# fundamentalvision/BEVFormer

Hardware: NVIDIA H100
Metric: BEV queries/sec (bevformer_base 200x200x256, 6 cams) fwd+bwd (higher is better)
Workload: dtype bf16

## Files before the change

### bevformer_b200/_lib.py

```python
from __future__ import annotations

import ctypes
import os
import threading

from . import build as _build

_lock = threading.Lock()
_lib = None

c_void_p, c_int, c_int64 = ctypes.c_void_p, ctypes.c_int, ctypes.c_int64

SIGNATURES = {
    "bevf_version": (c_int, []),
    "bevf_last_error": (ctypes.c_char_p, []),
    "bevf_launch_count": (c_int64, []),
    "bevf_msda_forward": (c_int, [c_void_p, c_int, c_void_p, c_void_p, c_void_p, c_void_p,
                                  c_void_p, c_int] + [c_int] * 7 + [c_void_p]),
    "bevf_msda_backward": (c_int, [c_void_p, c_int, c_void_p, c_void_p, c_void_p, c_void_p,
                                   c_void_p, c_int, c_void_p, c_void_p, c_void_p] + [c_int] * 7
                           + [c_void_p]),
    "bevf_msda_rows_forward": (c_int, [c_void_p, c_int, c_void_p, c_void_p, c_void_p, c_void_p,
                                       c_void_p, c_int, c_void_p] + [c_int] * 7 + [c_void_p]),
    "bevf_msda_rows_backward": (c_int, [c_void_p, c_int, c_void_p, c_void_p, c_void_p, c_void_p,
# ... 58 lines not shown
    "bevf_sca_combine_forward": (c_int, [c_void_p] * 4 + [c_int] * 6 + [c_void_p]),
    "bevf_sca_combine_backward": (c_int, [c_void_p] * 4 + [c_int] * 5 + [c_void_p]),
    "bevf_linear_forward": (c_int, [c_void_p] * 3 + [c_int] + [c_void_p] * 2
                            + [c_int, c_int64, c_int, c_int, c_int, c_void_p]),
    "bevf_flatten_feats": (c_int, [c_void_p] * 4 + [c_int] * 7 + [c_void_p]),
    "bevf_linear_dgrad": (c_int, [c_void_p] * 3 + [c_int64, c_int, c_int, c_void_p]),
    "bevf_linear_dgrad_acc": (c_int, [c_void_p] * 4 + [c_int64, c_int, c_int, c_void_p]),
    "bevf_linear_wgrad": (c_int, [c_void_p] * 4 + [c_int64, c_int, c_int, c_void_p]),
    "bevf_linear_wgrad_workspace_bytes": (c_int64, [c_int64, c_int, c_int]),
    "bevf_linear_wgrad_out": (c_int, [c_void_p] * 4 + [c_int, c_void_p, c_int64, c_int64, c_int, c_int,
                                                      c_void_p]),
    "bevf_sum_tensors": (c_int, [c_void_p, c_int, c_void_p, c_int64, c_int, c_void_p]),
    "bevf_linear_wgrad_into": (c_int, [c_void_p] * 5 + [c_int64, c_int64, c_int, c_int, c_void_p]),
    "bevf_linear_forward_dt": (c_int, [c_void_p] * 3 + [c_int] + [c_void_p] * 2
                               + [c_int, c_int64, c_int, c_int, c_int, c_int, c_void_p]),
    "bevf_linear_dgrad_dt": (c_int, [c_void_p] * 3 + [c_int64, c_int, c_int, c_int, c_void_p]),
    "bevf_linear_dgrad_acc_dt": (c_int, [c_void_p] * 4 + [c_int64, c_int, c_int, c_int, c_void_p]),
    "bevf_linear_wgrad_dt": (c_int, [c_void_p] * 4 + [c_int64, c_int, c_int, c_int, c_void_p]),
    "bevf_linear_wgrad_out_dt": (c_int, [c_void_p] * 4 + [c_int, c_void_p, c_int64, c_int64, c_int, c_int, c_int,
                                                         c_void_p]),
    "bevf_linear_wgrad_into_dt": (c_int, [c_void_p] * 5 + [c_int64, c_int64, c_int, c_int, c_int, c_void_p]),
    "bevf_colsum": (c_int, [c_void_p, c_void_p, c_int64, c_int, c_int, c_void_p]),
    "bevf_colsum_workspace_bytes": (c_int64, [c_int64, c_int]),
    "bevf_colsum_det": (c_int, [c_void_p, c_void_p, c_void_p, c_int64, c_int64, c_int, c_int, c_void_p]),
    "bevf_dropout_inplace": (c_int, [c_void_p, c_int64, ctypes.c_float, ctypes.c_uint64, c_void_p, c_int,
                                     c_void_p]),
    "bevf_relu_dropout_backward": (c_int, [c_void_p, c_void_p, c_void_p, c_int64, ctypes.c_float, c_int,
                                           c_void_p]),
    "bevf_point_sampling": (c_int, [c_void_p, c_void_p, c_void_p, ctypes.c_float, ctypes.c_float,
                                    c_void_p, c_void_p] + [c_int] * 5 + [c_void_p]),
# ... 64 lines not shown
```

### bevformer_b200/csrc/gemm.cu

```cuda
#include <cuda.h>

#include <cstdlib>
#include <cstring>
#include <type_traits>

#include "common.cuh"
#include "wgmma.cuh"

namespace bevf {

constexpr int kBM = 128;
constexpr int kBK = 64;
constexpr int kGemmThreads = 384;
constexpr int kChunk = 64 * 128;
constexpr int kMaxStages = 6;

__device__ __forceinline__ float load_bias(const void *bias, int dt, int col) {
    if (dt == BEVF_DTYPE_BF16) return __bfloat162float(reinterpret_cast<const bf16 *>(bias)[col]);
    if (dt == BEVF_DTYPE_F16) return __half2float(reinterpret_cast<const __half *>(bias)[col]);
    return reinterpret_cast<const float *>(bias)[col];
}

struct GemmParams {
    int M, N;
// ... 185 lines not shown
                if (p.red) {
                    float *dst = reinterpret_cast<float *>(p.y) + off;
                    asm volatile("red.global.add.v2.f32 [%0], {%1, %2};" ::"l"(dst), "f"(v0), "f"(v1) : "memory");
                } else if (p.out_f32) {
                    *reinterpret_cast<float2 *>(reinterpret_cast<float *>(p.y) + off) = make_float2(v0, v1);
                } else {
                    *reinterpret_cast<uint32_t *>(reinterpret_cast<TE *>(p.y) + off) = St16<TE>::pack(v0, v1);
                }
            }
        }
    }
}

constexpr int kWsRows = 64;
constexpr int kWsBoxBytes = 64 * 128;
constexpr int kWsStageMax = 4 * kWsBoxBytes;
constexpr int kWsWeightMax = 128 * 1024;

struct WsParams {
    int M, N, R;
    int tiles_m, tiles_n, groups;
    int stages;
    int stg_bytes;
    int relu;
    const void *bias;
    int bias_dt;
    int addend;
    int out_f32;
};

__device__ __forceinline__ void tma_store_2d(const CUtensorMap *map, const void *src, int c0, int c1) {
    asm volatile("cp.async.bulk.tensor.2d.global.shared::cta.bulk_group [%0, {%2, %3}], [%1];"
                 ::"l"(map), "r"(smem_u32(src)), "r"(c0), "r"(c1) : "memory");
}

template <int BN, bool kBmn, typename TE>
__global__ void __launch_bounds__(kGemmThreads, 1)
gemm_ws_wgmma(const __grid_constant__ CUtensorMap map_a, const __grid_constant__ CUtensorMap map_w,
              const __grid_constant__ CUtensorMap map_y, const __grid_constant__ CUtensorMap map_add,
              const WsParams p) {
    static_assert(BN == 64 || BN == 128 || BN == 256, "tile width");
    extern __shared__ __align__(1024) uint8_t smem_raw[];
    uint8_t *smem = reinterpret_cast<uint8_t *>((reinterpret_cast<uintptr_t>(smem_raw) + 1023) & ~uintptr_t(1023));
    const int kblocks = p.R / kBK;
    const int w_bytes = kblocks * BN * 128;
    uint8_t *sw = smem;
    uint8_t *stg0 = sw + w_bytes;
    uint8_t *ring0 = stg0 + 2 * p.stg_bytes;
    uint64_t *bars = reinterpret_cast<uint64_t *>(ring0 + 2 * p.stages * kWsBoxBytes);
    uint64_t *w_full = bars;
    uint64_t *full = bars + 1, *empty = full + 2 * kMaxStages;
    uint64_t *add_full = empty + 2 * kMaxStages, *stg_empty = add_full + 2;
    float *sbias = reinterpret_cast<float *>(stg_empty + 2);

    const int wg = threadIdx.x >> 7, warp = threadIdx.x >> 5, lane = threadIdx.x & 31;
    const int tn = blockIdx.x % p.tiles_n, g = blockIdx.x / p.tiles_n;
    const int t_begin = (int)((int64_t)g * p.tiles_m / p.groups);
    const int t_end = (int)((int64_t)(g + 1) * p.tiles_m / p.groups);
    const int col0 = tn * BN;

    if (threadIdx.x == 0) {
        asm volatile("prefetch.tensormap [%0];" ::"l"(&map_a) : "memory");
        asm volatile("prefetch.tensormap [%0];" ::"l"(&map_w) : "memory");
        asm volatile("prefetch.tensormap [%0];" ::"l"(&map_y) : "memory");
        mbar_init(w_full, 1);
        for (int i = 0; i < 2 * kMaxStages; ++i) { mbar_init(&full[i], 1); mbar_init(&empty[i], 4); }
        for (int i = 0; i < 2; ++i) { mbar_init(&add_full[i], 1); mbar_init(&stg_empty[i], 1); }
        asm volatile("fence.mbarrier_init.release.cluster;" ::: "memory");
    }
    __syncthreads();

    if (wg == 0) {
        asm volatile("setmaxnreg.dec.sync.aligned.u32 40;\n" ::: "memory");
        if (warp < 2 && lane == 0) {
            const int c = warp;
            if (c == 0) {
                const int chunks = kBmn ? min(BN / 64, (p.N - col0 + 63) / 64) : 1;
                mbar_expect_tx(w_full, (uint32_t)(kblocks * (kBmn ? chunks * kChunk : BN * 128)));
                for (int kb = 0; kb < kblocks; ++kb) {
                    uint8_t *dst = sw + (size_t)kb * BN * 128;
                    if (!kBmn) {
                        tma_load_2d(dst, &map_w, w_full, kb * kBK, col0);
                    } else {
                        for (int ch = 0; ch < chunks; ++ch)
                            tma_load_2d(dst + ch * kChunk, &map_w, w_full, col0 + ch * 64, kb * kBK);
                    }
                }
            }
            uint8_t *ring = ring0 + (size_t)c * p.stages * kWsBoxBytes, *stg = stg0 + (size_t)c * p.stg_bytes;
            uint64_t *f = full + c * kMaxStages, *e = empty + c * kMaxStages;
            const int add_boxes = min(BN / 64, (p.N - col0 + 63) / 64);
            int s = 0; uint32_t ph = 0, t = 0;
            for (int tm = t_begin + c; tm < t_end; tm += 2, ++t) {
                for (int kb = 0; kb < kblocks; ++kb) {
                    mbar_wait(&e[s], ph ^ 1);
                    mbar_expect_tx(&f[s], (uint32_t)kWsBoxBytes);
                    tma_load_2d(ring + (size_t)s * kWsBoxBytes, &map_a, &f[s], kb * kBK, tm * kWsRows);
                    if (++s == p.stages) { s = 0; ph ^= 1; }
                }
                if (p.addend) {
                    if (t > 0) mbar_wait(&stg_empty[c], (t - 1) & 1);
                    mbar_expect_tx(&add_full[c], (uint32_t)(add_boxes * kWsBoxBytes));
                    for (int b = 0; b < add_boxes; ++b)
                        tma_load_2d(stg + b * kWsBoxBytes, &map_add, &add_full[c], col0 + b * 64, tm * kWsRows);
                }
            }
        }
        return;
    }
    asm volatile("setmaxnreg.inc.sync.aligned.u32 232;\n" ::: "memory");

    const int cw = wg - 1, w4 = warp & 3;
    const bool leader = (threadIdx.x & 127) == 0;
    uint8_t *ring = ring0 + (size_t)cw * p.stages * kWsBoxBytes, *stg = stg0 + (size_t)cw * p.stg_bytes;
    uint64_t *f = full + cw * kMaxStages, *e = empty + cw * kMaxStages;
    constexpr int kF32PassCols = BN > 128 ? 128 : BN;
    const int passes = p.out_f32 ? BN / kF32PassCols : 1;
    const uint32_t sw_base = smem_u32(sw);
    constexpr uint64_t db_step = kBmn ? 128 : 2;
    float acc[BN / 2];
    for (int i = threadIdx.x - 128; i < BN; i += 256) {
        const int col = col0 + i;
        float b = 0.f;
        if (p.bias && col < p.N) b = load_bias(p.bias, p.bias_dt, col);
        sbias[i] = b;
    }
    asm volatile("bar.sync 3, 256;" ::: "memory");
    mbar_wait(w_full, 0);
    int s = 0; uint32_t ph = 0, t = 0;
    for (int tm = t_begin + cw; tm < t_end; tm += 2, ++t) {
        int prev = -1;
        for (int kb = 0; kb < kblocks; ++kb) {
            mbar_wait(&f[s], ph);
            const uint64_t da = smem_desc_sw128(smem_u32(ring + (size_t)s * kWsBoxBytes), 0);
            const uint64_t db = smem_desc_sw128(sw_base + (uint32_t)(kb * BN * 128), kChunk);
            wgmma_fence();
#pragma unroll
            for (int k = 0; k < kBK / 16; ++k)
                Wgmma<BN, 0, kBmn, TE>::run(acc, da + 2 * k, db + db_step * k, (kb | k) != 0);
            wgmma_commit();
            if (prev >= 0) {
                asm volatile("wgmma.wait_group.sync.aligned 1;" ::: "memory");
                __syncwarp();
                if (lane == 0) mbar_arrive(&e[prev]);
            }
            prev = s;
            if (++s == p.stages) { s = 0; ph ^= 1; }
// ... 10 lines not shown
            const float2 bv = *reinterpret_cast<const float2 *>(sbias + 8 * j + cq);
            const float b0 = bv.x, b1 = bv.y;
#pragma unroll
            for (int h = 0; h < 2; ++h) {
                float v0 = acc[4 * j + 2 * h] + b0, v1 = acc[4 * j + 2 * h + 1] + b1;
                if (p.relu) { v0 = fmaxf(v0, 0.f); v1 = fmaxf(v1, 0.f); }
                if (p.addend) {
                    const int r = r0 + 8 * h;
                    const uint32_t a2 = *reinterpret_cast<const uint32_t *>(
                        stg + (j >> 3) * kWsBoxBytes + r * 128 + (((j & 7) ^ (r & 7)) << 4) + 2 * cq);
                    v0 += St16<TE>::lo(a2); v1 += St16<TE>::hi(a2);
                }
                acc[4 * j + 2 * h] = v0; acc[4 * j + 2 * h + 1] = v1;
            }
        }
#pragma unroll
        for (int pass = 0; pass < 2; ++pass) {
            if (pass == passes) break;
            asm volatile("bar.sync %0, 128;" ::"r"(1 + cw) : "memory");
#pragma unroll
            for (int j = 0; j < BN / 8; ++j) {
#pragma unroll
                for (int h = 0; h < 2; ++h) {
                    const int r = r0 + 8 * h;
                    const float v0 = acc[4 * j + 2 * h], v1 = acc[4 * j + 2 * h + 1];
                    if (p.out_f32) {
                        if (j * 8 / kF32PassCols != pass) continue;
                        const int jj = j - pass * (kF32PassCols / 8);
                        const int unit = 2 * (jj & 3) + (cq >> 2);
                        *reinterpret_cast<float2 *>(stg + (jj >> 2) * kWsBoxBytes + r * 128 + ((unit ^ (r & 7)) << 4) +
                                                    4 * (cq & 3)) = make_float2(v0, v1);
                    } else {
                        *reinterpret_cast<uint32_t *>(stg + (j >> 3) * kWsBoxBytes + r * 128 +
                                                      (((j & 7) ^ (r & 7)) << 4) + 2 * cq) = St16<TE>::pack(v0, v1);
                    }
                }
            }
            asm volatile("fence.proxy.async.shared::cta;" ::: "memory");
            asm volatile("bar.sync %0, 128;" ::"r"(1 + cw) : "memory");
            if (leader) {
                const int cols_per_box = p.out_f32 ? 32 : 64, pc0 = col0 + pass * (BN / passes);
                for (int b = 0; b < BN / passes / cols_per_box && pc0 + b * cols_per_box < p.N; ++b)
                    tma_store_2d(&map_y, stg + b * kWsBoxBytes, pc0 + b * cols_per_box, tm * kWsRows);
                asm volatile("cp.async.bulk.commit_group;" ::: "memory");
                asm volatile("cp.async.bulk.wait_group.read 0;" ::: "memory");
            }
        }
        if (leader && p.addend) mbar_arrive(&stg_empty[cw]);
    }
    if (leader) asm volatile("cp.async.bulk.wait_group 0;" ::: "memory");
}

template <typename TO, bool kAcc = false>
__global__ void __launch_bounds__(256)
wgrad_reduce_kernel(const float *__restrict__ ws, const float *__restrict__ ws_b, TO *__restrict__ dw,
                    TO *__restrict__ db, int N, int K, int n_pad, int splits) {
    static_assert(!kAcc || sizeof(TO) == 4, "accumulation into fp32 only");
    const int kv = K / 4;
    const long long t = (long long)blockIdx.x * blockDim.x + threadIdx.x;
    const long long total = (long long)N * kv;
    if (t < total) {
        const int n = (int)(t / kv), c = (int)(t % kv) * 4;
        float4 a = make_float4(0.f, 0.f, 0.f, 0.f);
// ... 46 lines not shown
    const uint32_t esz = f32 ? 4 : 2;
    cuuint64_t dims[2] = {cols, rows};
    cuuint64_t strides[1] = {cols * esz};
    cuuint32_t box[2] = {128 / esz, box_rows};
    cuuint32_t estr[2] = {1, 1};
    const CUtensorMapDataType ty = f32 ? CU_TENSOR_MAP_DATA_TYPE_FLOAT32
                                 : dt == BEVF_DTYPE_F16 ? CU_TENSOR_MAP_DATA_TYPE_FLOAT16 : CU_TENSOR_MAP_DATA_TYPE_BFLOAT16;
    CUresult r = encode(map, ty, 2,
                        const_cast<void *>(ptr), dims,
                        strides, box, estr, CU_TENSOR_MAP_INTERLEAVE_NONE,
                        CU_TENSOR_MAP_SWIZZLE_128B, CU_TENSOR_MAP_L2_PROMOTION_L2_256B,
                        CU_TENSOR_MAP_FLOAT_OOB_FILL_NONE);
    return r == CUDA_SUCCESS ? 0 : (int)r;
}

template <int BN, bool kAmn, bool kBmn, typename TE>
static int launch_gemm(const char *who, const CUtensorMap &map_a, const CUtensorMap &map_b, GemmParams p,
                       cudaStream_t st) {
    constexpr int kStageBytes = kBM * 128 + BN * 128;
    int stages = (227 * 1024 - 1024 - 256) / kStageBytes;
    if (stages > kMaxStages) stages = kMaxStages;
    p.stages = stages;
    const size_t smem = 1024 + (size_t)stages * kStageBytes + 2 * kMaxStages * 8;
    static bool configured = false;
    if (!configured) {
        if (cudaFuncSetAttribute(gemm_bf16_wgmma<BN, kAmn, kBmn, TE>, cudaFuncAttributeMaxDynamicSharedMemorySize,
                                 (int)smem) != cudaSuccess) {
            cudaGetLastError();
            return fail("%s: cannot reserve shared memory for the GEMM", who);
        }
        configured = true;
    }
    const int units = ((p.M + kBM - 1) / kBM) * ((p.N + BN - 1) / BN) * p.splits;
    const int grid = units < device_sms() ? units : device_sms();
    gemm_bf16_wgmma<BN, kAmn, kBmn, TE><<<grid, kGemmThreads, smem, st>>>(map_a, map_b, p);
    return check_launch(who);
}

static int ws_block(int N, int R) {
    int bn = 256;
    while (bn > 64 && (bn * R * 2 > kWsWeightMax || bn / 2 >= N)) bn /= 2;
    return bn * R * 2 <= kWsWeightMax ? bn : 0;
}

template <int BN, bool kBmn, typename TE>
static int launch_ws(const char *who, const CUtensorMap &map_a, const CUtensorMap &map_w, const CUtensorMap &map_y,
                     const CUtensorMap &map_add, WsParams p, cudaStream_t st) {
    constexpr int kSmemMax = 227 * 1024;
    constexpr int kBarBytes = (1 + 4 * kMaxStages + 4) * 8 + BN * 4;
    p.stg_bytes = kWsRows * BN * (p.out_f32 ? 4 : 2);
    if (p.stg_bytes > kWsStageMax) p.stg_bytes = kWsStageMax;
    const int w_bytes = p.R * BN * 2;
    int stages = (kSmemMax - 1024 - kBarBytes - w_bytes - 2 * p.stg_bytes) / (2 * kWsBoxBytes);
    if (stages > kMaxStages) stages = kMaxStages;
    if (stages < 2) return fail("%s: no room for a two-stage A ring next to the weight tile", who);
    p.stages = stages;
    const size_t smem = 1024 + (size_t)w_bytes + 2 * p.stg_bytes + 2 * (size_t)stages * kWsBoxBytes + kBarBytes;
    static bool configured = false;
    if (!configured) {
        if (cudaFuncSetAttribute(gemm_ws_wgmma<BN, kBmn, TE>, cudaFuncAttributeMaxDynamicSharedMemorySize, kSmemMax) !=
            cudaSuccess) {
            cudaGetLastError();
            return fail("%s: cannot reserve shared memory for the GEMM", who);
        }
        configured = true;
    }
    p.tiles_m = (p.M + kWsRows - 1) / kWsRows;
    p.tiles_n = (p.N + BN - 1) / BN;
    p.groups = device_sms() / p.tiles_n;
    if (p.groups > p.tiles_m) p.groups = p.tiles_m;
    if (p.groups < 1) p.groups = 1;
    gemm_ws_wgmma<BN, kBmn, TE><<<p.groups * p.tiles_n, kGemmThreads, smem, st>>>(map_a, map_w, map_y, map_add, p);
    return check_launch(who);
}

template <typename TE> constexpr int dtype_of() { return std::is_same<TE, __half>::value ? BEVF_DTYPE_F16 : BEVF_DTYPE_BF16; }

template <typename TE>
static int linear_ws(const char *who, int bn, bool b_mn, const void *a, const void *w, const void *bias, int bias_dt,
                     const void *addend, void *y, bool out_f32, int M, int N, int R, int relu, cudaStream_t st) {
    constexpr int dt = dtype_of<TE>();
    CUtensorMap map_a, map_w, map_y, map_add;
    if (int e = make_map_2d(&map_a, a, (uint64_t)M, (uint64_t)R, kWsRows, dt))
        return fail("%s: cuTensorMapEncodeTiled(A) failed (%lld)", who, e);
    if (int e = b_mn ? make_map_2d(&map_w, w, (uint64_t)R, (uint64_t)N, 64, dt)
                     : make_map_2d(&map_w, w, (uint64_t)N, (uint64_t)R, (uint32_t)bn, dt))
        return fail("%s: cuTensorMapEncodeTiled(B) failed (%lld)", who, e);
    if (int e = make_map_2d(&map_y, y, (uint64_t)M, (uint64_t)N, kWsRows, out_f32 ? BEVF_DTYPE_F32 : dt))
        return fail("%s: cuTensorMapEncodeTiled(Y) failed (%lld)", who, e);
    map_add = map_y;
    if (addend)
        if (int e = make_map_2d(&map_add, addend, (uint64_t)M, (uint64_t)N, kWsRows, dt))
            return fail("%s: cuTensorMapEncodeTiled(addend) failed (%lld)", who, e);
    WsParams p;
    memset(&p, 0, sizeof(p));
    p.M = M; p.N = N; p.R = R;
    p.relu = relu; p.bias = bias; p.bias_dt = bias_dt;
    p.addend = addend != nullptr; p.out_f32 = out_f32;
    switch (bn * 2 + (int)b_mn) {
        case 512: return launch_ws<256, false, TE>(who, map_a, map_w, map_y, map_add, p, st);
        case 513: return launch_ws<256, true, TE>(who, map_a, map_w, map_y, map_add, p, st);
        case 256: return launch_ws<128, false, TE>(who, map_a, map_w, map_y, map_add, p, st);
        case 257: return launch_ws<128, true, TE>(who, map_a, map_w, map_y, map_add, p, st);
        case 128: return launch_ws<64, false, TE>(who, map_a, map_w, map_y, map_add, p, st);
        case 129: return launch_ws<64, true, TE>(who, map_a, map_w, map_y, map_add, p, st);
    }
    return fail("%s: no weight-stationary tile for this shape", who);
}

static GemmParams base_params(int M, int N, int R) {
    GemmParams p;
    memset(&p, 0, sizeof(p));
    p.M = M; p.N = N; p.R = R; p.rows_per_split = ((R + kBK - 1) / kBK) * kBK; p.splits = 1;
    p.ldy = N;
    return p;
}
// ... 3 lines not shown
using namespace bevf;

static bool operand_dtype_ok(int dtype) { return dtype == BEVF_DTYPE_BF16 || dtype == BEVF_DTYPE_F16; }

template <typename TE>
static int linear_dgrad_impl(const char *who, const void *dy, const void *w, const void *addend, void *dx, int64_t M,
                             int N, int K, void *stream) {
    constexpr int dt = dtype_of<TE>();
    if (M < 0 || N <= 0 || K <= 0) return fail("%s: bad dimension", who);
    if (M == 0) return 0;
    if (!dy || !w || !dx) return fail("%s: null pointer argument", who);
    if (N % kBK != 0 || K % 64 != 0) return fail("%s: N and K must be multiples of 64 (got %lld, %lld)", who, N, K);
    if (M >= (1ll << 31)) return fail("%s: M too large", who);
    if (!aligned16(dy) || !aligned16(w) || !aligned16(dx)) return fail("%s: pointers must be 16-byte aligned", who);
    cudaStream_t st = (cudaStream_t)stream;
    if (int bn = ws_block(K, N))
        return linear_ws<TE>(who, bn, true, dy, w, nullptr, BEVF_DTYPE_F32, addend, dx, false, (int)M, K, N, 0, st);
    CUtensorMap map_a, map_b;
    if (int e = make_map_2d(&map_a, dy, (uint64_t)M, (uint64_t)N, kBM, dt))
        return fail("%s: cuTensorMapEncodeTiled(A) failed (%lld)", who, e);
    if (int e = make_map_2d(&map_b, w, (uint64_t)N, (uint64_t)K, 64, dt))
        return fail("%s: cuTensorMapEncodeTiled(B) failed (%lld)", who, e);
    GemmParams p = base_params((int)M, K, N);
    p.addend = addend;
    p.y = dx;
    return K % 128 == 0 ? launch_gemm<128, false, true, TE>(who, map_a, map_b, p, st)
                        : launch_gemm<64, false, true, TE>(who, map_a, map_b, p, st);
}

static int linear_dgrad_dispatch(const char *who, const void *dy, const void *w, const void *addend, void *dx,
                                 int64_t M, int N, int K, int dtype, void *stream) {
// ... 28 lines not shown
                               void *stream) {
    constexpr int dt = dtype_of<TE>();
    if (M < 0 || N <= 0 || K <= 0) return fail("%s: bad dimension", who);
    if (M == 0) return 0;
    if (!x || !w || !y) return fail("%s: null pointer argument", who);
    if (K % kBK != 0) return fail("%s: K must be a multiple of 64 (got %lld)", who, K);
    if (N % 16 != 0) return fail("%s: N must be a multiple of 16 (got %lld)", who, N);
    if (M >= (1ll << 31)) return fail("%s: M too large", who);
    if (!aligned16(x) || !aligned16(w) || !aligned16(y) || (bias && !aligned16(bias)) ||
        (residual && !aligned16(residual)))
        return fail("%s: pointers must be 16-byte aligned", who);
    if (y_dtype != dt && y_dtype != BEVF_DTYPE_F32) return fail("%s: unsupported dtype code", who);
    if (bias && bias_dtype != dt && bias_dtype != BEVF_DTYPE_F32)
        return fail("%s: unsupported bias dtype code", who);
    cudaStream_t st = (cudaStream_t)stream;
    if (int bn = ws_block(N, K))
        return linear_ws<TE>(who, bn, false, x, w, bias, bias_dtype, residual, y, y_dtype == BEVF_DTYPE_F32, (int)M, N,
                             K, relu, st);
    const bool wide = N > 64;
    CUtensorMap map_a, map_b;
    if (int e = make_map_2d(&map_a, x, (uint64_t)M, (uint64_t)K, kBM, dt))
        return fail("%s: cuTensorMapEncodeTiled(A) failed (%lld)", who, e);
    if (int e = make_map_2d(&map_b, w, (uint64_t)N, (uint64_t)K, wide ? 128 : 64, dt))
        return fail("%s: cuTensorMapEncodeTiled(B) failed (%lld)", who, e);
    GemmParams p = base_params((int)M, N, K);
    p.relu = relu; p.bias = bias; p.bias_dt = bias_dtype;
    p.addend = residual;
    p.y = y; p.out_f32 = y_dtype == BEVF_DTYPE_F32;
    return wide ? launch_gemm<128, false, false, TE>(who, map_a, map_b, p, st)
                : launch_gemm<64, false, false, TE>(who, map_a, map_b, p, st);
}
// ... 2 lines not shown
                                      const void *residual, void *y, int y_dtype, int64_t M, int N, int K, int relu,
                                      int dtype, void *stream) {
    const char *who = "bevf_linear_forward_dt";
    if (dtype == BEVF_DTYPE_F16)
        return linear_forward_impl<__half>(who, x, w, bias, bias_dtype, residual, y, y_dtype, M, N, K, relu, stream);
    if (dtype == BEVF_DTYPE_BF16)
        return linear_forward_impl<bf16>(who, x, w, bias, bias_dtype, residual, y, y_dtype, M, N, K, relu, stream);
    return fail("%s: unsupported operand dtype code (bf16 or fp16)", who);
}

extern "C" int bevf_linear_forward(const void *x, const void *w, const void *bias, int bias_dtype,
                                   const void *residual, void *y, int y_dtype, int64_t M, int N, int K,
                                   int relu, void *stream) {
    return linear_forward_impl<bf16>("bevf_linear_forward", x, w, bias, bias_dtype, residual, y, y_dtype, M, N, K,
                                     relu, stream);
}

static void wgrad_plan(int64_t M, int N, int K, int &bn, int &splits, int &rows, int &n_pad) {
    bn = K % 128 == 0 ? 128 : 64;
    const int tiles_m = (N + kBM - 1) / kBM;
    const int tiles = tiles_m * (K / bn);
    splits = (device_sms() + tiles - 1) / tiles;
    rows = (int)((M + splits - 1) / splits);
    rows = ((rows + 63) / 64) * 64;
    splits = (int)((M + rows - 1) / rows);
    n_pad = tiles_m * kBM;
}

template <typename TE>
static int launch_wgrad(const char *who, const void *dy, const void *x, GemmParams p, int bn, cudaStream_t st) {
// ... 113 lines not shown
```

### bevformer_b200/ops.py

```python
from __future__ import annotations

import os
import warnings

import torch
from torch.autograd.function import Function, once_differentiable

from . import _lib

F32, BF16, F16 = 0, 1, 2
_DT = {torch.float32: F32, torch.bfloat16: BF16, torch.float16: F16}
TC_DTYPES = (torch.bfloat16, torch.float16)


def deterministic() -> bool:
    return torch.are_deterministic_algorithms_enabled()


def alert_not_deterministic(name: str) -> None:
    if not torch.are_deterministic_algorithms_enabled():
        return
    msg = (f"{name} does not have a deterministic implementation, but you set "
           "'torch.use_deterministic_algorithms(True)'.")
    if torch.is_deterministic_algorithms_warn_only_enabled():
# ... 942 lines not shown
    _need_cuda(x, "x")
    if x.dtype not in TC_DTYPES or weight.dtype != x.dtype:
        raise RuntimeError("linear_tc: x and weight must be both bfloat16 or both float16")
    K = x.shape[-1]
    N = weight.shape[0]
    M = x.numel() // K
    w = weight.contiguous()
    bq, bdt = (None, F32) if bias is None else _param_ptr(bias, x.dtype)
    res = None if residual is None else residual.contiguous()
    out_dtype = out_dtype or x.dtype
    y = torch.empty(x.shape[:-1] + (N,), device=x.device, dtype=out_dtype)
    lib = _lib.load()
    with torch.cuda.device(x.device):
        st = lib.bevf_linear_forward_dt(x.data_ptr(), w.data_ptr(), _ptr(bq), bdt, _ptr(res), y.data_ptr(),
                                        _DT[out_dtype], M, N, K, int(bool(relu)), _DT[x.dtype], _stream_ptr(x))
    _lib.check(st, lib)
    return y


def linear_dgrad_tc(dy, weight, addend=None):
    _need_cuda(dy, "dy")
    if dy.dtype not in TC_DTYPES or weight.dtype != dy.dtype or dy.shape[-1] != weight.shape[0]:
        raise RuntimeError("linear_dgrad_tc: dy (M,N) and weight (N,K) must be both bfloat16 or both float16")
    N, K = weight.shape
    if N % 64 or K % 64 or os.environ.get("BEVF_DGRAD", "mn") == "copy":
        dx = linear_tc(dy, weight.t().contiguous())
        return dx if addend is None else dx + addend.view(dx.shape)
    dy = dy.contiguous()
    w = weight.contiguous()
    M = dy.numel() // N
# ... 465 lines not shown
```

### bevformer_b200/plugin/linear.py

```python
from __future__ import annotations

import os

import torch
import torch.nn.functional as F
from torch.autograd.function import Function, once_differentiable

from .. import ops
from ..arena import arena_of


def _use_tc(x: torch.Tensor, weight: torch.Tensor) -> bool:
    return (x.is_cuda and x.dtype in ops.TC_DTYPES and weight.shape[1] % 64 == 0
            and weight.shape[0] % 16 == 0 and os.environ.get("BEVF_GEMM", "tc") != "cublas")


def stacked_head(weights, biases, x):
    from ..arena import stacked
    n, k = sum(w.shape[0] for w in weights), weights[0].shape[1]
    direct = (x.is_cuda and x.dtype in ops.TC_DTYPES and k % 64 == 0 and n % 16 == 0
              and os.environ.get("BEVF_GEMM", "tc") != "cublas")
    return stacked(weights, direct), stacked(biases, direct)


# ... 86 lines not shown


class _SharedInputProjections(Function):

    @staticmethod
    def forward(ctx, state, x, *wb):
        xc = x.contiguous()
        ws, outs, meta = [], [], []
        aux = ops.aux_stream(xc.device) if os.environ.get("BEVF_AUX_PROJ", "0") == "1" else None
        main = torch.cuda.current_stream(xc.device) if aux is not None else None
        ready = []
        if aux is not None:
            ev = torch.cuda.Event()
            ev.record(main)
            aux.wait_event(ev)
        for i in range(0, len(wb), 2):
            w = wb[i].to(xc.dtype)
            ws.append(w)
            if aux is None:
                outs.append(ops.linear_tc(xc, w, wb[i + 1], None, False, xc.dtype))
            else:
                with torch.cuda.stream(aux):
                    o = ops.linear_tc(xc, w, wb[i + 1], None, False, xc.dtype)
                    e = torch.cuda.Event()
                    e.record(aux)
                o.record_stream(main)
                outs.append(o)
                ready.append(e)
            meta.append((wb[i].dtype, None if wb[i + 1] is None else wb[i + 1].dtype))
        if aux is not None:
            xc.record_stream(aux)
        state["ready"] = ready
        ctx.save_for_backward(xc, *ws)
        ctx.set_materialize_grads(False)
        ctx.meta = meta
        ctx.arenas = [_arena_ctx(wb[i], wb[i + 1]) for i in range(0, len(wb), 2)]
        ctx.state = state
        state.update(x2=xc.reshape(-1, xc.shape[-1]), ws=ws, meta=meta, arenas=ctx.arenas,
                     early=[None] * len(ws), need_dx=x.requires_grad)
        return tuple(outs)

    @staticmethod
    def early(state, l, dy):
        ar = state["arenas"][l]
# ... 216 lines not shown
```

### include/bevformer_b200.h

```cpp
#ifndef BEVFORMER_B200_H_
#define BEVFORMER_B200_H_

#include <stdint.h>

#ifdef __cplusplus
extern "C" {
#endif

#define BEVF_ABI_VERSION 3

#if defined(__GNUC__)
#define BEVF_API __attribute__((visibility("default")))
#else
#define BEVF_API
#endif

enum bevf_dtype { BEVF_DTYPE_F32 = 0, BEVF_DTYPE_BF16 = 1, BEVF_DTYPE_F16 = 2 };

BEVF_API int bevf_version(void);

BEVF_API const char *bevf_last_error(void);

BEVF_API int64_t bevf_launch_count(void);

// ... 200 lines not shown
BEVF_API int bevf_dropout_inplace(void *x, int64_t n, float p, uint64_t seed, const uint64_t *seed_base,
                                  int dtype, void *stream);
BEVF_API int bevf_relu_dropout_backward(const void *dy, const void *h, void *out, int64_t n, float scale,
                                        int dtype, void *stream);

BEVF_API int64_t bevf_linear_wgrad_workspace_bytes(int64_t M, int N, int K);
BEVF_API int bevf_linear_wgrad_out(const void *dy, const void *x, void *dw, void *db, int grad_dtype,
                                   void *workspace, int64_t workspace_bytes, int64_t M, int N, int K,
                                   void *stream);
BEVF_API int bevf_linear_wgrad_into(const void *dy, const void *x, float *dw, float *db, void *workspace,
                                    int64_t workspace_bytes, int64_t M, int N, int K, void *stream);

BEVF_API int bevf_linear_forward_dt(const void *x, const void *w, const void *bias, int bias_dtype,
                                    const void *residual, void *y, int y_dtype, int64_t M, int N, int K,
                                    int relu, int dtype, void *stream);
BEVF_API int bevf_linear_dgrad_dt(const void *dy, const void *w, void *dx, int64_t M, int N, int K, int dtype,
                                  void *stream);
BEVF_API int bevf_linear_dgrad_acc_dt(const void *dy, const void *w, const void *addend, void *dx, int64_t M,
                                      int N, int K, int dtype, void *stream);
BEVF_API int bevf_linear_wgrad_dt(const void *dy, const void *x, float *dw, float *db, int64_t M, int N,
                                  int K, int dtype, void *stream);
BEVF_API int bevf_linear_wgrad_out_dt(const void *dy, const void *x, void *dw, void *db, int grad_dtype,
                                      void *workspace, int64_t workspace_bytes, int64_t M, int N, int K,
                                      int dtype, void *stream);
BEVF_API int bevf_linear_wgrad_into_dt(const void *dy, const void *x, float *dw, float *db, void *workspace,
                                       int64_t workspace_bytes, int64_t M, int N, int K, int dtype,
                                       void *stream);

BEVF_API int bevf_attn_forward(const void *q, int64_t ldq, const void *k, int64_t ldk, const void *v, int64_t ldv,
                               void *out, int64_t ldo, float *lse, int nq, int nk, int bs, int heads, int head_dim,
// ... 33 lines not shown
```

Measured before the change: 1.748 million.

## Batch same-input linears into one stacked weight-stationary GEMM with per-k-block weight barriers

Several linears that share one input are now computed by a single weight-stationary GEMM over concatenated weights. The output goes through a 3D TMA map that writes each layer's slice into a stacked [layers, M, N] tensor, replacing one launch per linear. The weight tile now gets one mbarrier per k-block, so compute can begin before the whole weight tile has landed. The epilogue no longer waits for the TMA store right after each tile, and the BN=256 variant is dropped in favour of smem-based stage sizing. This applies only when no aux stream is in use, and it adds a torch.cat of the weights on every call.

New measurement: 1.782 million, median of 6. 1.9% higher.

```diff
diff --git a/bevformer_b200/_lib.py b/bevformer_b200/_lib.py
--- a/bevformer_b200/_lib.py
+++ b/bevformer_b200/_lib.py
@@ -96,6 +96,8 @@
     "bevf_linear_wgrad_into": (c_int, [c_void_p] * 5 + [c_int64, c_int64, c_int, c_int, c_void_p]),
     "bevf_linear_forward_dt": (c_int, [c_void_p] * 3 + [c_int] + [c_void_p] * 2
                                + [c_int, c_int64, c_int, c_int, c_int, c_int, c_void_p]),
+    "bevf_linear_forward_stacked_dt": (c_int, [c_void_p] * 3 + [c_int, c_void_p, c_int64, c_int, c_int, c_int, c_int,
+                                                                 c_void_p]),
     "bevf_linear_dgrad_dt": (c_int, [c_void_p] * 3 + [c_int64, c_int, c_int, c_int, c_void_p]),
     "bevf_linear_dgrad_acc_dt": (c_int, [c_void_p] * 4 + [c_int64, c_int, c_int, c_int, c_void_p]),
     "bevf_linear_wgrad_dt": (c_int, [c_void_p] * 4 + [c_int64, c_int, c_int, c_int, c_void_p]),
diff --git a/bevformer_b200/csrc/gemm.cu b/bevformer_b200/csrc/gemm.cu
--- a/bevformer_b200/csrc/gemm.cu
+++ b/bevformer_b200/csrc/gemm.cu
@@ -223,8 +223,9 @@
 
 constexpr int kWsRows = 64;
 constexpr int kWsBoxBytes = 64 * 128;
-constexpr int kWsStageMax = 4 * kWsBoxBytes;
 constexpr int kWsWeightMax = 128 * 1024;
+constexpr int kWsMaxKBlocks = kWsWeightMax / (64 * 128);
+constexpr int kWsMaxStages = 8;
 
 struct WsParams {
     int M, N, R;
@@ -236,11 +237,12 @@
     int bias_dt;
     int addend;
     int out_f32;
+    int n_layer;
 };
 
-__device__ __forceinline__ void tma_store_2d(const CUtensorMap *map, const void *src, int c0, int c1) {
-    asm volatile("cp.async.bulk.tensor.2d.global.shared::cta.bulk_group [%0, {%2, %3}], [%1];"
-                 ::"l"(map), "r"(smem_u32(src)), "r"(c0), "r"(c1) : "memory");
+__device__ __forceinline__ void tma_store_3d(const CUtensorMap *map, const void *src, int c0, int c1, int c2) {
+    asm volatile("cp.async.bulk.tensor.3d.global.shared::cta.bulk_group [%0, {%2, %3, %4}], [%1];"
+                 ::"l"(map), "r"(smem_u32(src)), "r"(c0), "r"(c1), "r"(c2) : "memory");
 }
 
 template <int BN, bool kBmn, typename TE>
@@ -248,7 +250,7 @@
 gemm_ws_wgmma(const __grid_constant__ CUtensorMap map_a, const __grid_constant__ CUtensorMap map_w,
               const __grid_constant__ CUtensorMap map_y, const __grid_constant__ CUtensorMap map_add,
               const WsParams p) {
-    static_assert(BN == 64 || BN == 128 || BN == 256, "tile width");
+    static_assert(BN == 64 || BN == 128, "tile width");
     extern __shared__ __align__(1024) uint8_t smem_raw[];
     uint8_t *smem = reinterpret_cast<uint8_t *>((reinterpret_cast<uintptr_t>(smem_raw) + 1023) & ~uintptr_t(1023));
     const int kblocks = p.R / kBK;
@@ -258,8 +260,8 @@
     uint8_t *ring0 = stg0 + 2 * p.stg_bytes;
     uint64_t *bars = reinterpret_cast<uint64_t *>(ring0 + 2 * p.stages * kWsBoxBytes);
     uint64_t *w_full = bars;
-    uint64_t *full = bars + 1, *empty = full + 2 * kMaxStages;
-    uint64_t *add_full = empty + 2 * kMaxStages, *stg_empty = add_full + 2;
+    uint64_t *full = bars + kWsMaxKBlocks, *empty = full + 2 * kWsMaxStages;
+    uint64_t *add_full = empty + 2 * kWsMaxStages, *stg_empty = add_full + 2;
     float *sbias = reinterpret_cast<float *>(stg_empty + 2);
 
     const int wg = threadIdx.x >> 7, warp = threadIdx.x >> 5, lane = threadIdx.x & 31;
@@ -272,8 +274,8 @@
         asm volatile("prefetch.tensormap [%0];" ::"l"(&map_a) : "memory");
         asm volatile("prefetch.tensormap [%0];" ::"l"(&map_w) : "memory");
         asm volatile("prefetch.tensormap [%0];" ::"l"(&map_y) : "memory");
-        mbar_init(w_full, 1);
-        for (int i = 0; i < 2 * kMaxStages; ++i) { mbar_init(&full[i], 1); mbar_init(&empty[i], 4); }
+        for (int i = 0; i < kblocks; ++i) mbar_init(&w_full[i], 1);
+        for (int i = 0; i < 2 * kWsMaxStages; ++i) { mbar_init(&full[i], 1); mbar_init(&empty[i], 4); }
         for (int i = 0; i < 2; ++i) { mbar_init(&add_full[i], 1); mbar_init(&stg_empty[i], 1); }
         asm volatile("fence.mbarrier_init.release.cluster;" ::: "memory");
     }
@@ -285,19 +287,19 @@
             const int c = warp;
             if (c == 0) {
                 const int chunks = kBmn ? min(BN / 64, (p.N - col0 + 63) / 64) : 1;
-                mbar_expect_tx(w_full, (uint32_t)(kblocks * (kBmn ? chunks * kChunk : BN * 128)));
                 for (int kb = 0; kb < kblocks; ++kb) {
                     uint8_t *dst = sw + (size_t)kb * BN * 128;
+                    mbar_expect_tx(&w_full[kb], (uint32_t)(kBmn ? chunks * kChunk : BN * 128));
                     if (!kBmn) {
-                        tma_load_2d(dst, &map_w, w_full, kb * kBK, col0);
+                        tma_load_2d(dst, &map_w, &w_full[kb], kb * kBK, col0);
                     } else {
                         for (int ch = 0; ch < chunks; ++ch)
-                            tma_load_2d(dst + ch * kChunk, &map_w, w_full, col0 + ch * 64, kb * kBK);
+                            tma_load_2d(dst + ch * kChunk, &map_w, &w_full[kb], col0 + ch * 64, kb * kBK);
                     }
                 }
             }
             uint8_t *ring = ring0 + (size_t)c * p.stages * kWsBoxBytes, *stg = stg0 + (size_t)c * p.stg_bytes;
-            uint64_t *f = full + c * kMaxStages, *e = empty + c * kMaxStages;
+            uint64_t *f = full + c * kWsMaxStages, *e = empty + c * kWsMaxStages;
             const int add_boxes = min(BN / 64, (p.N - col0 + 63) / 64);
             int s = 0; uint32_t ph = 0, t = 0;
             for (int tm = t_begin + c; tm < t_end; tm += 2, ++t) {
@@ -322,9 +324,7 @@
     const int cw = wg - 1, w4 = warp & 3;
     const bool leader = (threadIdx.x & 127) == 0;
     uint8_t *ring = ring0 + (size_t)cw * p.stages * kWsBoxBytes, *stg = stg0 + (size_t)cw * p.stg_bytes;
-    uint64_t *f = full + cw * kMaxStages, *e = empty + cw * kMaxStages;
-    constexpr int kF32PassCols = BN > 128 ? 128 : BN;
-    const int passes = p.out_f32 ? BN / kF32PassCols : 1;
+    uint64_t *f = full + cw * kWsMaxStages, *e = empty + cw * kWsMaxStages;
     const uint32_t sw_base = smem_u32(sw);
     constexpr uint64_t db_step = kBmn ? 128 : 2;
     float acc[BN / 2];
@@ -335,11 +335,11 @@
         sbias[i] = b;
     }
     asm volatile("bar.sync 3, 256;" ::: "memory");
-    mbar_wait(w_full, 0);
     int s = 0; uint32_t ph = 0, t = 0;
     for (int tm = t_begin + cw; tm < t_end; tm += 2, ++t) {
         int prev = -1;
         for (int kb = 0; kb < kblocks; ++kb) {
+            if (tm < t_begin + 2) mbar_wait(&w_full[kb], 0);
             mbar_wait(&f[s], ph);
             const uint64_t da = smem_desc_sw128(smem_u32(ring + (size_t)s * kWsBoxBytes), 0);
             const uint64_t db = smem_desc_sw128(sw_base + (uint32_t)(kb * BN * 128), kChunk);
@@ -380,39 +380,37 @@
                 acc[4 * j + 2 * h] = v0; acc[4 * j + 2 * h + 1] = v1;
             }
         }
-#pragma unroll
-        for (int pass = 0; pass < 2; ++pass) {
-            if (pass == passes) break;
-            asm volatile("bar.sync %0, 128;" ::"r"(1 + cw) : "memory");
-#pragma unroll
-            for (int j = 0; j < BN / 8; ++j) {
-#pragma unroll
-                for (int h = 0; h < 2; ++h) {
-                    const int r = r0 + 8 * h;
-                    const float v0 = acc[4 * j + 2 * h], v1 = acc[4 * j + 2 * h + 1];
-                    if (p.out_f32) {
-                        if (j * 8 / kF32PassCols != pass) continue;
-                        const int jj = j - pass * (kF32PassCols / 8);
-                        const int unit = 2 * (jj & 3) + (cq >> 2);
-                        *reinterpret_cast<float2 *>(stg + (jj >> 2) * kWsBoxBytes + r * 128 + ((unit ^ (r & 7)) << 4) +
-                                                    4 * (cq & 3)) = make_float2(v0, v1);
-                    } else {
-                        *reinterpret_cast<uint32_t *>(stg + (j >> 3) * kWsBoxBytes + r * 128 +
-                                                      (((j & 7) ^ (r & 7)) << 4) + 2 * cq) = St16<TE>::pack(v0, v1);
-                    }
+        if (leader) asm volatile("cp.async.bulk.wait_group.read 0;" ::: "memory");
+        asm volatile("bar.sync %0, 128;" ::"r"(1 + cw) : "memory");
+#pragma unroll
+        for (int j = 0; j < BN / 8; ++j) {
+#pragma unroll
+            for (int h = 0; h < 2; ++h) {
+                const int r = r0 + 8 * h;
+                const float v0 = acc[4 * j + 2 * h], v1 = acc[4 * j + 2 * h + 1];
+                if (p.out_f32) {
+                    const int unit = 2 * (j & 3) + (cq >> 2);
+                    *reinterpret_cast<float2 *>(stg + (j >> 2) * kWsBoxBytes + r * 128 + ((unit ^ (r & 7)) << 4) +
+                                                4 * (cq & 3)) = make_float2(v0, v1);
+                } else {
+                    *reinterpret_cast<uint32_t *>(stg + (j >> 3) * kWsBoxBytes + r * 128 +
+                                                  (((j & 7) ^ (r & 7)) << 4) + 2 * cq) = St16<TE>::pack(v0, v1);
                 }
             }
-            asm volatile("fence.proxy.async.shared::cta;" ::: "memory");
-            asm volatile("bar.sync %0, 128;" ::"r"(1 + cw) : "memory");
-            if (leader) {
-                const int cols_per_box = p.out_f32 ? 32 : 64, pc0 = col0 + pass * (BN / passes);
-                for (int b = 0; b < BN / passes / cols_per_box && pc0 + b * cols_per_box < p.N; ++b)
-                    tma_store_2d(&map_y, stg + b * kWsBoxBytes, pc0 + b * cols_per_box, tm * kWsRows);
-                asm volatile("cp.async.bulk.commit_group;" ::: "memory");
-                asm volatile("cp.async.bulk.wait_group.read 0;" ::: "memory");
-            }
-        }
-        if (leader && p.addend) mbar_arrive(&stg_empty[cw]);
+        }
+        asm volatile("fence.proxy.async.shared::cta;" ::: "memory");
+        asm volatile("bar.sync %0, 128;" ::"r"(1 + cw) : "memory");
+        if (leader) {
+            const int cols_per_box = p.out_f32 ? 32 : 64;
+            const int layer = col0 / p.n_layer, lc0 = col0 - layer * p.n_layer;
+            for (int b = 0; b < BN / cols_per_box && col0 + b * cols_per_box < p.N; ++b)
+                tma_store_3d(&map_y, stg + b * kWsBoxBytes, lc0 + b * cols_per_box, tm * kWsRows, layer);
+            asm volatile("cp.async.bulk.commit_group;" ::: "memory");
+        }
+        if (leader && p.addend) {
+            asm volatile("cp.async.bulk.wait_group.read 0;" ::: "memory");
+            mbar_arrive(&stg_empty[cw]);
+        }
     }
     if (leader) asm volatile("cp.async.bulk.wait_group 0;" ::: "memory");
 }
@@ -489,6 +487,22 @@
     return r == CUDA_SUCCESS ? 0 : (int)r;
 }
 
+static int make_map_3d(CUtensorMap *map, const void *ptr, uint64_t layers, uint64_t rows, uint64_t cols, int dt) {
+    EncodeTiledFn encode = encode_tiled_fn();
+    if (!encode) return -1;
+    const bool f32 = dt == BEVF_DTYPE_F32;
+    const uint32_t esz = f32 ? 4 : 2;
+    cuuint64_t dims[3] = {cols, rows, layers};
+    cuuint64_t strides[2] = {cols * esz, rows * cols * esz};
+    cuuint32_t box[3] = {128 / esz, 64, 1};
+    cuuint32_t estr[3] = {1, 1, 1};
+    const CUtensorMapDataType ty = f32 ? CU_TENSOR_MAP_DATA_TYPE_FLOAT32
+                                 : dt == BEVF_DTYPE_F16 ? CU_TENSOR_MAP_DATA_TYPE_FLOAT16 : CU_TENSOR_MAP_DATA_TYPE_BFLOAT16;
+    CUresult r = encode(map, ty, 3, const_cast<void *>(ptr), dims, strides, box, estr, CU_TENSOR_MAP_INTERLEAVE_NONE,
+                        CU_TENSOR_MAP_SWIZZLE_128B, CU_TENSOR_MAP_L2_PROMOTION_L2_256B, CU_TENSOR_MAP_FLOAT_OOB_FILL_NONE);
+    return r == CUDA_SUCCESS ? 0 : (int)r;
+}
+
 template <int BN, bool kAmn, bool kBmn, typename TE>
 static int launch_gemm(const char *who, const CUtensorMap &map_a, const CUtensorMap &map_b, GemmParams p,
                        cudaStream_t st) {
@@ -512,29 +526,33 @@
     return check_launch(who);
 }
 
-static int ws_block(int N, int R) {
-    int bn = 256;
-    while (bn > 64 && (bn * R * 2 > kWsWeightMax || bn / 2 >= N)) bn /= 2;
-    return bn * R * 2 <= kWsWeightMax ? bn : 0;
+constexpr int kWsSmemMax = 227 * 1024;
+static int ws_stg_bytes(int bn, bool out_f32) { return kWsRows * bn * (out_f32 ? 4 : 2); }
+static int ws_fixed_bytes(int bn, int R, bool out_f32) {
+    return 1024 + R * bn * 2 + 2 * ws_stg_bytes(bn, out_f32) + (kWsMaxKBlocks + 4 * kWsMaxStages + 4) * 8 + bn * 4;
+}
+static int ws_stages(int bn, int R, bool out_f32) {
+    const int stages = (kWsSmemMax - ws_fixed_bytes(bn, R, out_f32)) / (2 * kWsBoxBytes);
+    return stages < kWsMaxStages ? stages : kWsMaxStages;
+}
+
+static int ws_block(int N, int R, bool out_f32) {
+    if (64 * R * 2 > kWsWeightMax) return 0;
+    if (N > 64 && 128 * R * 2 <= kWsWeightMax && ws_stages(128, R, out_f32) >= 4) return 128;
+    return 64;
 }
 
 template <int BN, bool kBmn, typename TE>
 static int launch_ws(const char *who, const CUtensorMap &map_a, const CUtensorMap &map_w, const CUtensorMap &map_y,
                      const CUtensorMap &map_add, WsParams p, cudaStream_t st) {
-    constexpr int kSmemMax = 227 * 1024;
-    constexpr int kBarBytes = (1 + 4 * kMaxStages + 4) * 8 + BN * 4;
-    p.stg_bytes = kWsRows * BN * (p.out_f32 ? 4 : 2);
-    if (p.stg_bytes > kWsStageMax) p.stg_bytes = kWsStageMax;
-    const int w_bytes = p.R * BN * 2;
-    int stages = (kSmemMax - 1024 - kBarBytes - w_bytes - 2 * p.stg_bytes) / (2 * kWsBoxBytes);
-    if (stages > kMaxStages) stages = kMaxStages;
-    if (stages < 2) return fail("%s: no room for a two-stage A ring next to the weight tile", who);
-    p.stages = stages;
-    const size_t smem = 1024 + (size_t)w_bytes + 2 * p.stg_bytes + 2 * (size_t)stages * kWsBoxBytes + kBarBytes;
+    p.stg_bytes = ws_stg_bytes(BN, p.out_f32);
+    p.stages = ws_stages(BN, p.R, p.out_f32);
+    if (p.stages < 2) return fail("%s: no room for a two-stage A ring next to the weight tile", who);
+    const size_t smem = (size_t)ws_fixed_bytes(BN, p.R, p.out_f32) + 2 * (size_t)p.stages * kWsBoxBytes;
     static bool configured = false;
     if (!configured) {
-        if (cudaFuncSetAttribute(gemm_ws_wgmma<BN, kBmn, TE>, cudaFuncAttributeMaxDynamicSharedMemorySize, kSmemMax) !=
-            cudaSuccess) {
+        if (cudaFuncSetAttribute(gemm_ws_wgmma<BN, kBmn, TE>, cudaFuncAttributeMaxDynamicSharedMemorySize,
+                                 kWsSmemMax) != cudaSuccess) {
             cudaGetLastError();
             return fail("%s: cannot reserve shared memory for the GEMM", who);
         }
@@ -553,7 +571,9 @@
 
 template <typename TE>
 static int linear_ws(const char *who, int bn, bool b_mn, const void *a, const void *w, const void *bias, int bias_dt,
-                     const void *addend, void *y, bool out_f32, int M, int N, int R, int relu, cudaStream_t st) {
+                     const void *addend, void *y, bool out_f32, int M, int N, int R, int relu, cudaStream_t st,
+                     int n_layer = 0) {
+    if (n_layer == 0) n_layer = N;
     constexpr int dt = dtype_of<TE>();
     CUtensorMap map_a, map_w, map_y, map_add;
     if (int e = make_map_2d(&map_a, a, (uint64_t)M, (uint64_t)R, kWsRows, dt))
@@ -561,7 +581,8 @@
     if (int e = b_mn ? make_map_2d(&map_w, w, (uint64_t)R, (uint64_t)N, 64, dt)
                      : make_map_2d(&map_w, w, (uint64_t)N, (uint64_t)R, (uint32_t)bn, dt))
         return fail("%s: cuTensorMapEncodeTiled(B) failed (%lld)", who, e);
-    if (int e = make_map_2d(&map_y, y, (uint64_t)M, (uint64_t)N, kWsRows, out_f32 ? BEVF_DTYPE_F32 : dt))
+    if (int e = make_map_3d(&map_y, y, (uint64_t)(N / n_layer), (uint64_t)M, (uint64_t)n_layer,
+                            out_f32 ? BEVF_DTYPE_F32 : dt))
         return fail("%s: cuTensorMapEncodeTiled(Y) failed (%lld)", who, e);
     map_add = map_y;
     if (addend)
@@ -571,10 +592,8 @@
     memset(&p, 0, sizeof(p));
     p.M = M; p.N = N; p.R = R;
     p.relu = relu; p.bias = bias; p.bias_dt = bias_dt;
-    p.addend = addend != nullptr; p.out_f32 = out_f32;
+    p.addend = addend != nullptr; p.out_f32 = out_f32; p.n_layer = n_layer;
     switch (bn * 2 + (int)b_mn) {
-        case 512: return launch_ws<256, false, TE>(who, map_a, map_w, map_y, map_add, p, st);
-        case 513: return launch_ws<256, true, TE>(who, map_a, map_w, map_y, map_add, p, st);
         case 256: return launch_ws<128, false, TE>(who, map_a, map_w, map_y, map_add, p, st);
         case 257: return launch_ws<128, true, TE>(who, map_a, map_w, map_y, map_add, p, st);
         case 128: return launch_ws<64, false, TE>(who, map_a, map_w, map_y, map_add, p, st);
@@ -608,7 +627,7 @@
     if (M >= (1ll << 31)) return fail("%s: M too large", who);
     if (!aligned16(dy) || !aligned16(w) || !aligned16(dx)) return fail("%s: pointers must be 16-byte aligned", who);
     cudaStream_t st = (cudaStream_t)stream;
-    if (int bn = ws_block(K, N))
+    if (int bn = ws_block(K, N, false))
         return linear_ws<TE>(who, bn, true, dy, w, nullptr, BEVF_DTYPE_F32, addend, dx, false, (int)M, K, N, 0, st);
     CUtensorMap map_a, map_b;
     if (int e = make_map_2d(&map_a, dy, (uint64_t)M, (uint64_t)N, kBM, dt))
@@ -667,7 +686,7 @@
     if (bias && bias_dtype != dt && bias_dtype != BEVF_DTYPE_F32)
         return fail("%s: unsupported bias dtype code", who);
     cudaStream_t st = (cudaStream_t)stream;
-    if (int bn = ws_block(N, K))
+    if (int bn = ws_block(N, K, y_dtype == BEVF_DTYPE_F32))
         return linear_ws<TE>(who, bn, false, x, w, bias, bias_dtype, residual, y, y_dtype == BEVF_DTYPE_F32, (int)M, N,
                              K, relu, st);
     const bool wide = N > 64;
@@ -700,6 +719,35 @@
                                    int relu, void *stream) {
     return linear_forward_impl<bf16>("bevf_linear_forward", x, w, bias, bias_dtype, residual, y, y_dtype, M, N, K,
                                      relu, stream);
+}
+
+template <typename TE>
+static int linear_stacked_impl(const char *who, const void *x, const void *w, const void *bias, int bias_dtype,
+                               void *y, int64_t M, int N, int K, int layers, void *stream) {
+    if (M < 0 || N <= 0 || K <= 0 || layers <= 0) return fail("%s: bad dimension", who);
+    if (M == 0) return 0;
+    if (!x || !w || !y) return fail("%s: null pointer argument", who);
+    if (K % kBK != 0 || N % 64 != 0) return fail("%s: K and N must be multiples of 64 (got %lld, %lld)", who, K, N);
+    if (M >= (1ll << 31) || (int64_t)N * layers >= (1ll << 31)) return fail("%s: M or layers x N too large", who);
+    if (!aligned16(x) || !aligned16(w) || !aligned16(y) || (bias && !aligned16(bias)))
+        return fail("%s: pointers must be 16-byte aligned", who);
+    if (bias && bias_dtype != dtype_of<TE>() && bias_dtype != BEVF_DTYPE_F32)
+        return fail("%s: unsupported bias dtype code", who);
+    int bn = ws_block(N * layers, K, false);
+    if (bn == 0) return fail("%s: reduction too long for the weight-stationary kernel (K = %lld)", who, K);
+    if (N % bn != 0) bn = 64;
+    return linear_ws<TE>(who, bn, false, x, w, bias, bias_dtype, nullptr, y, false, (int)M, N * layers, K, 0,
+                         (cudaStream_t)stream, N);
+}
+
+extern "C" int bevf_linear_forward_stacked_dt(const void *x, const void *w, const void *bias, int bias_dtype, void *y,
+                                              int64_t M, int N, int K, int layers, int dtype, void *stream) {
+    const char *who = "bevf_linear_forward_stacked_dt";
+    if (dtype == BEVF_DTYPE_F16)
+        return linear_stacked_impl<__half>(who, x, w, bias, bias_dtype, y, M, N, K, layers, stream);
+    if (dtype == BEVF_DTYPE_BF16)
+        return linear_stacked_impl<bf16>(who, x, w, bias, bias_dtype, y, M, N, K, layers, stream);
+    return fail("%s: unsupported operand dtype code (bf16 or fp16)", who);
 }
 
 static void wgrad_plan(int64_t M, int N, int K, int &bn, int &splits, int &rows, int &n_pad) {
diff --git a/bevformer_b200/ops.py b/bevformer_b200/ops.py
--- a/bevformer_b200/ops.py
+++ b/bevformer_b200/ops.py
@@ -980,6 +980,25 @@
     with torch.cuda.device(x.device):
         st = lib.bevf_linear_forward_dt(x.data_ptr(), w.data_ptr(), _ptr(bq), bdt, _ptr(res), y.data_ptr(),
                                         _DT[out_dtype], M, N, K, int(bool(relu)), _DT[x.dtype], _stream_ptr(x))
+    _lib.check(st, lib)
+    return y
+
+
+def linear_stacked_tc(x, weight, bias, layers):
+    _need_cuda(x, "x")
+    if x.dtype not in TC_DTYPES or weight.dtype != x.dtype:
+        raise RuntimeError("linear_stacked_tc: x and weight must be both bfloat16 or both float16")
+    K = x.shape[-1]
+    N = weight.shape[0] // layers
+    M = x.numel() // K
+    x = x.contiguous()
+    w = weight.contiguous()
+    bq, bdt = (None, F32) if bias is None else _param_ptr(bias, x.dtype)
+    y = torch.empty((layers,) + x.shape[:-1] + (N,), device=x.device, dtype=x.dtype)
+    lib = _lib.load()
+    with torch.cuda.device(x.device):
+        st = lib.bevf_linear_forward_stacked_dt(x.data_ptr(), w.data_ptr(), _ptr(bq), bdt, y.data_ptr(), M, N, K,
+                                                layers, _DT[x.dtype], _stream_ptr(x))
     _lib.check(st, lib)
     return y
 
diff --git a/bevformer_b200/plugin/linear.py b/bevformer_b200/plugin/linear.py
--- a/bevformer_b200/plugin/linear.py
+++ b/bevformer_b200/plugin/linear.py
@@ -124,20 +124,30 @@
             ev = torch.cuda.Event()
             ev.record(main)
             aux.wait_event(ev)
-        for i in range(0, len(wb), 2):
-            w = wb[i].to(xc.dtype)
-            ws.append(w)
-            if aux is None:
-                outs.append(ops.linear_tc(xc, w, wb[i + 1], None, False, xc.dtype))
-            else:
-                with torch.cuda.stream(aux):
-                    o = ops.linear_tc(xc, w, wb[i + 1], None, False, xc.dtype)
-                    e = torch.cuda.Event()
-                    e.record(aux)
-                o.record_stream(main)
-                outs.append(o)
-                ready.append(e)
-            meta.append((wb[i].dtype, None if wb[i + 1] is None else wb[i + 1].dtype))
+        n = wb[0].shape[0]
+        biases = wb[1::2]
+        if (aux is None and n % 64 == 0 and all(w.shape == wb[0].shape for w in wb[0::2])
+                and (all(b is None for b in biases) or all(b is not None for b in biases))):
+            w_all = torch.cat([w.to(xc.dtype) for w in wb[0::2]])
+            ws = list(w_all.split(n))
+            outs = list(ops.linear_stacked_tc(xc, w_all, None if biases[0] is None else torch.cat(biases),
+                                              len(ws)).unbind(0))
+            meta = [(w.dtype, None if b is None else b.dtype) for w, b in zip(wb[0::2], biases)]
+        else:
+            for i in range(0, len(wb), 2):
+                w = wb[i].to(xc.dtype)
+                ws.append(w)
+                if aux is None:
+                    outs.append(ops.linear_tc(xc, w, wb[i + 1], None, False, xc.dtype))
+                else:
+                    with torch.cuda.stream(aux):
+                        o = ops.linear_tc(xc, w, wb[i + 1], None, False, xc.dtype)
+                        e = torch.cuda.Event()
+                        e.record(aux)
+                    o.record_stream(main)
+                    outs.append(o)
+                    ready.append(e)
+                meta.append((wb[i].dtype, None if wb[i + 1] is None else wb[i + 1].dtype))
         if aux is not None:
             xc.record_stream(aux)
         state["ready"] = ready
diff --git a/include/bevformer_b200.h b/include/bevformer_b200.h
--- a/include/bevformer_b200.h
+++ b/include/bevformer_b200.h
@@ -238,6 +238,8 @@
 BEVF_API int bevf_linear_forward_dt(const void *x, const void *w, const void *bias, int bias_dtype,
                                     const void *residual, void *y, int y_dtype, int64_t M, int N, int K,
                                     int relu, int dtype, void *stream);
+BEVF_API int bevf_linear_forward_stacked_dt(const void *x, const void *w, const void *bias, int bias_dtype, void *y,
+                                            int64_t M, int N, int K, int layers, int dtype, void *stream);
 BEVF_API int bevf_linear_dgrad_dt(const void *dy, const void *w, void *dx, int64_t M, int N, int K, int dtype,
                                   void *stream);
 BEVF_API int bevf_linear_dgrad_acc_dt(const void *dy, const void *w, const void *addend, void *dx, int64_t M,
```
